# shenweichen/DeepCTR

Hardware: NVIDIA H100
Metric: samples/sec fwd+bwd DeepFM Criteo-synth (higher is better)
Workload: dtype f32

## Files before the change

deepctr_b200/csrc/embed.cu:

```cuda
#include <stdlib.h>
#include <cuda_bf16.h>
#include "common.cuh"

namespace b2ctr {

namespace farm {
__host__ __device__ constexpr uint64_t k0() { return 0xc3a5c85c97cb3127ULL; }
__host__ __device__ constexpr uint64_t k1() { return 0xb492b66fbe98f273ULL; }
__host__ __device__ constexpr uint64_t k2() { return 0x9ae16a3b2f90404fULL; }
__device__ __forceinline__ uint64_t rot(uint64_t v, int s) { return (v >> s) | (v << (64 - s)); }
__device__ __forceinline__ uint64_t shift_mix(uint64_t v) { return v ^ (v >> 47); }
__device__ __forceinline__ uint64_t fetch64(const unsigned char* p) {
  uint64_t r = 0;
#pragma unroll
  for (int i = 7; i >= 0; --i) r = (r << 8) | p[i];
  return r;
}
__device__ __forceinline__ uint64_t fetch32(const unsigned char* p) {
  return (uint64_t)p[0] | ((uint64_t)p[1] << 8) | ((uint64_t)p[2] << 16) | ((uint64_t)p[3] << 24);
}
__device__ __forceinline__ uint64_t hash_len16(uint64_t u, uint64_t v, uint64_t mul) {
  uint64_t a = (u ^ v) * mul;
  a ^= (a >> 47);
  uint64_t b = (v ^ a) * mul;
// ... 212 lines not shown
      V acc = vzero<VEC>();
      bool first = true;
      for (int t0 = 0; t0 < T; t0 += 4) {
        int64_t id[4];
        bool val[4];
        V x[4];
#pragma unroll
        for (int u = 0; u < 4; ++u) {
          const int t = t0 + u;
          id[u] = t < T ? lookup_id(ft, ibase + t) : 0;
          val[u] = t < T && pos_valid(ft, t, id[u], len);
        }
#pragma unroll
        for (int u = 0; u < 4; ++u) {
          const bool need = t0 + u < T && (val[u] || ft.pool == B2CTR_POOL_MAX);
          const bool ok = id_in_range(id[u], ft.vocab);
          if (need && !ok && e == 0) note_oob(fb.oob);
          x[u] = (need && ok) ? vload(ft.table + id[u] * dim + e, (V*)nullptr) : vzero<VEC>();
        }
#pragma unroll
        for (int u = 0; u < 4; ++u) {
          const int t = t0 + u;
          if (t >= T) break;
          V v = x[u];
          if (ft.weight_mode != B2CTR_WEIGHT_NONE) v = vmuls(v, pos_weight(ft, si, b, t, val[u]));
          if (ft.pool == B2CTR_POOL_MAX) {
            if (!val[u]) v = vsubs(v, 1e9f);
            acc = first ? v : vmax(acc, v);
            first = false;
          } else if (val[u]) {
            acc = vadd(acc, v);
          }
        }
      }
      if (ft.pool == B2CTR_POOL_MEAN) acc = vdivs(acc, __fadd_rn(si.L, 1e-8f));
      vstore(out + e, acc);
    }
  }
}

template <int G, int VEC>
__global__ void __launch_bounds__(256)
    embed_scatter_generic_kernel(const __grid_constant__ FeatBlock fb, int64_t batch, float scale) {
  using V = typename VecT<VEC>::T;
  constexpr int kGroups = 256 / G;
  const int lane = threadIdx.x % G;
  const unsigned gmask = G >= 32 ? 0xffffffffu : (((1u << (G & 31)) - 1u) << ((threadIdx.x & 31) / G * G));
  const int64_t ntasks = batch * fb.nfeat;
  for (int64_t task = (int64_t)blockIdx.x * kGroups + threadIdx.x / G; task < ntasks;
       task += (int64_t)gridDim.x * kGroups) {
    const int64_t b = task / fb.nfeat;
    const b2ctr_feature_t& ft = fb.f[task - b * fb.nfeat];
    const int dim = ft.dim, T = ft.maxlen;
    const float* gout = ft.out + b * ft.out_ld + ft.out_col;
    const int64_t ibase = b * ft.idx_stride;

    if (ft.pool == B2CTR_POOL_NONE) {
      for (int t = 0; t < T; ++t) {
        const int64_t id = lookup_id(ft, ibase + t);
        if (!id_in_range(id, ft.vocab)) continue;
        bool nz = false;
        for (int e = lane * VEC; e < dim; e += G * VEC) nz |= vnonzero(vload(gout + (int64_t)t * dim + e, (V*)nullptr));
        if (__ballot_sync(gmask, nz) == 0u) continue;
        float* row = ft.table + id * dim;
        for (int e = lane * VEC; e < dim; e += G * VEC)
          vred(row + e, vmuls(vload(gout + (int64_t)t * dim + e, (V*)nullptr), scale));
      }
      continue;
    }
    const int len = ft.mask_mode == B2CTR_MASK_LENGTH ? ft.len[b * lstride(ft)] : 0;
    const SeqInfo si = seq_info(ft, b);
    for (int e = lane * VEC; e < dim; e += G * VEC) {
      V g = vmuls(vload(gout + e, (V*)nullptr), scale);
      if (ft.pool == B2CTR_POOL_MEAN) g = vdivs(g, __fadd_rn(si.L, 1e-8f));
      if (ft.pool == B2CTR_POOL_MAX) {
        float gv[VEC], mx[VEC];
        int cnt[VEC];
        {
          float tmp[VEC];
          *reinterpret_cast<V*>(tmp) = g;
#pragma unroll
          for (int i = 0; i < VEC; ++i) { gv[i] = tmp[i]; mx[i] = -INFINITY; cnt[i] = 0; }
        }
        for (int pass = 0; pass < 2; ++pass) {
          for (int t = 0; t < T; ++t) {
            const int64_t id = lookup_id(ft, ibase + t);
            const bool valid = pos_valid(ft, t, id, len);
            const bool ok = id_in_range(id, ft.vocab);
            V xv = ok ? vload((ft.src_table ? ft.src_table : ft.table) + id * dim + e, (V*)nullptr) : vzero<VEC>();
            const float w = pos_weight(ft, si, b, t, valid);
            if (ft.weight_mode != B2CTR_WEIGHT_NONE) xv = vmuls(xv, w);
            if (!valid) xv = vsubs(xv, 1e9f);
            float xs[VEC];
            *reinterpret_cast<V*>(xs) = xv;
            if (pass == 0) {
#pragma unroll
              for (int i = 0; i < VEC; ++i) {
                if (xs[i] > mx[i]) { mx[i] = xs[i]; cnt[i] = 1; }
                else if (xs[i] == mx[i]) cnt[i]++;
              }
            } else {
#pragma unroll
              for (int i = 0; i < VEC; ++i)
                if (xs[i] == mx[i] && ok) red_add_f1(ft.table + id * dim + e + i, gv[i] / (float)cnt[i] * w);
            }
          }
        }
        continue;
      }
      for (int t = 0; t < T; ++t) {
        const int64_t id = lookup_id(ft, ibase + t);
        const bool valid = pos_valid(ft, t, id, len);
        if (!valid || !id_in_range(id, ft.vocab)) continue;
        V gt = g;
        if (ft.weight_mode != B2CTR_WEIGHT_NONE) gt = vmuls(gt, pos_weight(ft, si, b, t, true));
        vred(ft.table + id * dim + e, gt);
      }
    }
  }
}

constexpr int kUniMaxFeat = 64;
struct UniParams {
  float* table[kUniMaxFeat];
  float* lin[kUniMaxFeat];
  const void* idx[kUniMaxFeat];
  int64_t idx_stride[kUniMaxFeat];
  int64_t vocab[kUniMaxFeat];
  unsigned long long* oob;
  const float* dense;
  float* x;
  float* linear;
  float* fm;
  int64_t ldx;
  int64_t dense_ld;
  int64_t x_cols;
  uint64_t fm_mask;
  int32_t nfeat;
  int32_t ndense;
  int32_t dim;
  int32_t idx_dtype;
  int32_t has_lin;
  int32_t l2_hints;
  int32_t store_grads;
  float* const* peer_tab;
  float* const* peer_lin;
  int32_t world;
  int32_t wshift;
  __nv_bfloat16* xp_hi;
  __nv_bfloat16* xp_lo;
  int64_t xp_pitch;
};

__device__ __forceinline__ void store_planes4(const UniParams& p, int64_t off, float4 v) {
  const __nv_bfloat16 h0 = __float2bfloat16_rn(v.x), h1 = __float2bfloat16_rn(v.y);
  const __nv_bfloat16 h2 = __float2bfloat16_rn(v.z), h3 = __float2bfloat16_rn(v.w);
  const __nv_bfloat16 l0 = __float2bfloat16_rn(v.x - __bfloat162float(h0));
  const __nv_bfloat16 l1 = __float2bfloat16_rn(v.y - __bfloat162float(h1));
  const __nv_bfloat16 l2 = __float2bfloat16_rn(v.z - __bfloat162float(h2));
  const __nv_bfloat16 l3 = __float2bfloat16_rn(v.w - __bfloat162float(h3));
  uint2 h, l;
  h.x = (uint32_t)__bfloat16_as_ushort(h0) | ((uint32_t)__bfloat16_as_ushort(h1) << 16);
  h.y = (uint32_t)__bfloat16_as_ushort(h2) | ((uint32_t)__bfloat16_as_ushort(h3) << 16);
  l.x = (uint32_t)__bfloat16_as_ushort(l0) | ((uint32_t)__bfloat16_as_ushort(l1) << 16);
  l.y = (uint32_t)__bfloat16_as_ushort(l2) | ((uint32_t)__bfloat16_as_ushort(l3) << 16);
  *reinterpret_cast<uint2*>(p.xp_hi + off) = h;
  *reinterpret_cast<uint2*>(p.xp_lo + off) = l;
}

__device__ __forceinline__ float4 ld_peer_f4(const float* p) {
  float4 r;
  asm volatile("ld.global.L1::no_allocate.v4.f32 {%0,%1,%2,%3}, [%4];"
               : "=f"(r.x), "=f"(r.y), "=f"(r.z), "=f"(r.w)
               : "l"(p));
  return r;
}
__device__ __forceinline__ float ld_peer_f1(const float* p) {
  float r;
  asm volatile("ld.global.L1::no_allocate.f32 %0, [%1];" : "=f"(r) : "l"(p));
  return r;
}
__device__ __forceinline__ void red_peer_f4(float* p, float4 v) {
  asm volatile("red.relaxed.sys.global.add.v4.f32 [%0], {%1,%2,%3,%4};" ::"l"(p), "f"(v.x), "f"(v.y), "f"(v.z),
               "f"(v.w)
               : "memory");
}
__device__ __forceinline__ void red_peer_f1(float* p, float v) {
  asm volatile("red.relaxed.sys.global.add.f32 [%0], %1;" ::"l"(p), "f"(v) : "memory");
}
__device__ __forceinline__ float* shard_row(float* const* tabs, const UniParams& p, int f, int64_t id, int width) {
  const int64_t own = id & (int64_t)(p.world - 1);
  return tabs[(int64_t)f * p.world + own] + (id >> p.wshift) * width;
}

__device__ __forceinline__ int64_t uni_id(const UniParams& p, int f, int64_t b) {
  return load_idx(p.idx[f], b * p.idx_stride[f], p.idx_dtype);
}

template <int LPR, bool SHARD, bool PLANES>
__global__ void __launch_bounds__(256, (SHARD || PLANES) ? 3 : 4)
    gather_uniform_fwd_kernel(const __grid_constant__ UniParams p, int64_t batch) {
  constexpr int RPI = 32 / LPR;
  constexpr int U = 7;
  const int lane = threadIdx.x & 31;
  const int slot = lane / LPR, chunk = lane % LPR;
  const int F = p.nfeat, dim = p.dim;
  const bool hints = p.l2_hints != 0;
  const uint64_t pol_keep = l2_policy_evict_last(), pol_stream = l2_policy_evict_first();
  const int64_t nwarps = (int64_t)gridDim.x * (blockDim.x >> 5);
  int64_t b = (int64_t)blockIdx.x * (blockDim.x >> 5) + (threadIdx.x >> 5);
  auto checked = [&](int f, int64_t bb) -> int64_t {
    if (bb >= batch || f >= F) return 0;
    const int64_t id = uni_id(p, f, bb);
    if (id_in_range(id, p.vocab[f])) return id;
    note_oob(p.oob);
    return -1;
  };
  int64_t id0 = checked(lane, b);
  int64_t id1 = checked(lane + 32, b);
  for (; b < batch; b += nwarps) {
    const int64_t bn = b + nwarps;
    const int64_t nid0 = checked(lane, bn);
    const int64_t nid1 = checked(lane + 32, bn);
    float* xrow = p.x + b * p.ldx;
    float4 s = make_float4(0.f, 0.f, 0.f, 0.f);
    float q = 0.f;
    for (int f0 = 0; f0 < F; f0 += U * RPI) {
      float4 v[U];
#pragma unroll
      for (int u = 0; u < U; ++u) {
        const int f = f0 + u * RPI + slot;
        const int fs = f < F ? f : 0;
        const int64_t ida = __shfl_sync(0xffffffffu, id0, fs & 31);
        const int64_t idb = __shfl_sync(0xffffffffu, id1, fs & 31);
        const int64_t id = fs < 32 ? ida : idb;
        if (f < F) {
          if (id < 0) {
            v[u] = make_float4(0.f, 0.f, 0.f, 0.f);
          } else if (SHARD) {
            v[u] = ld_peer_f4(shard_row(p.peer_tab, p, f, id, dim) + chunk * 4);
          } else {
            const float* src = p.table[f] + id * dim + chunk * 4;
            v[u] = hints ? ldg_stream_f4_pol(src, pol_stream) : ldg_stream_f4(src);
          }
        }
      }
#pragma unroll
      for (int u = 0; u < U; ++u) {
        const int f = f0 + u * RPI + slot;
        if (f < F) {
          if (hints) stg_stream_f4_pol(xrow + (int64_t)f * dim + chunk * 4, v[u], pol_stream);
          else stg_stream_f4(xrow + (int64_t)f * dim + chunk * 4, v[u]);
          if (PLANES) store_planes4(p, b * p.xp_pitch + (int64_t)f * dim + chunk * 4, v[u]);
          if ((p.fm_mask >> f) & 1ull) {
            s.x += v[u].x; s.y += v[u].y; s.z += v[u].z; s.w += v[u].w;
            q += v[u].x * v[u].x + v[u].y * v[u].y + v[u].z * v[u].z + v[u].w * v[u].w;
          }
        }
      }
    }
    if (p.fm != nullptr) {
#pragma unroll
      for (int o = LPR; o < 32; o <<= 1) {
        s.x += __shfl_xor_sync(0xffffffffu, s.x, o);
        s.y += __shfl_xor_sync(0xffffffffu, s.y, o);
        s.z += __shfl_xor_sync(0xffffffffu, s.z, o);
        s.w += __shfl_xor_sync(0xffffffffu, s.w, o);
      }
      float sq = slot == 0 ? (s.x * s.x + s.y * s.y + s.z * s.z + s.w * s.w) : 0.f;
      sq = warp_sum(sq);
      q = warp_sum(q);
      if (lane == 0) p.fm[b] = 0.5f * (sq - q);
    }
    if (p.linear != nullptr) {
      float l = 0.f;
      if (p.has_lin) {
        const bool ok0 = lane < F && id0 >= 0;
        const bool ok1 = lane + 32 < F && id1 >= 0;
        if (SHARD) {
          if (ok0) l += ld_peer_f1(shard_row(p.peer_lin, p, lane, id0, 1));
          if (ok1) l += ld_peer_f1(shard_row(p.peer_lin, p, lane + 32, id1, 1));
        } else {
          if (ok0) l += hints ? ldg_f1_pol(p.lin[lane] + id0, pol_keep) : p.lin[lane][id0];
          if (ok1) l += hints ? ldg_f1_pol(p.lin[lane + 32] + id1, pol_keep) : p.lin[lane + 32][id1];
        }
      }
      l = warp_sum(l);
      if (lane == 0) p.linear[b] = l;
    }
    const int64_t c0 = (int64_t)F * dim;
    for (int64_t c = c0 + lane; c < p.x_cols; c += 32) {
      const int j = (int)(c - c0);
      xrow[c] = j < p.ndense ? p.dense[b * p.dense_ld + j] : 0.f;
    }
    if (PLANES) {
      for (int64_t c = c0 + lane; c < p.xp_pitch; c += 32) {
        const int j = (int)(c - c0);
        const float v = j < p.ndense ? p.dense[b * p.dense_ld + j] : 0.f;
        const __nv_bfloat16 h = __float2bfloat16_rn(v);
        p.xp_hi[b * p.xp_pitch + c] = h;
        p.xp_lo[b * p.xp_pitch + c] = __float2bfloat16_rn(v - __bfloat162float(h));
      }
    }
    id0 = nid0;
    id1 = nid1;
  }
}

template <int LPR, bool SHARD>
__global__ void __launch_bounds__(256, SHARD ? 2 : 3)
    scatter_uniform_bwd_kernel(const __grid_constant__ UniParams p, const float* __restrict__ dx,
                               const float* __restrict__ dfm, const float* __restrict__ dlinear,
                               float scale, float lin_scale, int64_t batch) {
  constexpr int RPI = 32 / LPR;
  constexpr int U = 4;
  const int lane = threadIdx.x & 31;
  const int slot = lane / LPR, chunk = lane % LPR;
  const int F = p.nfeat, dim = p.dim;
  const bool hints = p.l2_hints != 0;
  const uint64_t pol_keep = l2_policy_evict_last(), pol_stream = l2_policy_evict_first();
  const int64_t nwarps = (int64_t)gridDim.x * (blockDim.x >> 5);
  int64_t b = (int64_t)blockIdx.x * (blockDim.x >> 5) + (threadIdx.x >> 5);
  auto checked = [&](int f, int64_t bb) -> int64_t {
    if (bb >= batch || f >= F) return 0;
    const int64_t id = uni_id(p, f, bb);
    return id_in_range(id, p.vocab[f]) ? id : -1;
  };
  int64_t id0 = checked(lane, b);
  int64_t id1 = checked(lane + 32, b);
  for (; b < batch; b += nwarps) {
    const int64_t bn = b + nwarps;
    const int64_t nid0 = checked(lane, bn);
    const int64_t nid1 = checked(lane + 32, bn);
    const float* xrow = p.x + b * p.ldx;
    const float* dxrow = dx ? dx + b * p.ldx : nullptr;
    const float gfm = dfm ? dfm[b] : 0.f;
    float4 s = make_float4(0.f, 0.f, 0.f, 0.f);
    if (dfm) {
      for (int f0 = 0; f0 < F; f0 += U * RPI) {
        float4 v[U];
#pragma unroll
        for (int u = 0; u < U; ++u) {
          const int f = f0 + u * RPI + slot;
          v[u] = make_float4(0.f, 0.f, 0.f, 0.f);
          if (f < F && ((p.fm_mask >> f) & 1ull))
            v[u] = *reinterpret_cast<const float4*>(xrow + (int64_t)f * dim + chunk * 4);
        }
#pragma unroll
        for (int u = 0; u < U; ++u) { s.x += v[u].x; s.y += v[u].y; s.z += v[u].z; s.w += v[u].w; }
      }
#pragma unroll
      for (int o = LPR; o < 32; o <<= 1) {
        s.x += __shfl_xor_sync(0xffffffffu, s.x, o);
        s.y += __shfl_xor_sync(0xffffffffu, s.y, o);
        s.z += __shfl_xor_sync(0xffffffffu, s.z, o);
        s.w += __shfl_xor_sync(0xffffffffu, s.w, o);
      }
    }
    for (int f0 = 0; f0 < F; f0 += U * RPI) {
      float4 g[U], xv[U];
#pragma unroll
      for (int u = 0; u < U; ++u) {
        const int f = f0 + u * RPI + slot;
        g[u] = make_float4(0.f, 0.f, 0.f, 0.f);
        xv[u] = g[u];
        if (f < F) {
          const int64_t off = (int64_t)f * dim + chunk * 4;
          if (dxrow) g[u] = hints ? ldg_stream_f4_pol(dxrow + off, pol_stream) : ldg_stream_f4(dxrow + off);
          if (dfm && ((p.fm_mask >> f) & 1ull)) xv[u] = *reinterpret_cast<const float4*>(xrow + off);
        }
      }
#pragma unroll
      for (int u = 0; u < U; ++u) {
        const int f = f0 + u * RPI + slot;
        const int fs = f < F ? f : 0;
        const int64_t ida = __shfl_sync(0xffffffffu, id0, fs & 31);
        const int64_t idb = __shfl_sync(0xffffffffu, id1, fs & 31);
        const int64_t id = fs < 32 ? ida : idb;
        if (f < F && id >= 0) {
          float4 r = g[u];
          if (dfm && ((p.fm_mask >> f) & 1ull)) {
            r.x += gfm * (s.x - xv[u].x);
            r.y += gfm * (s.y - xv[u].y);
            r.z += gfm * (s.z - xv[u].z);
            r.w += gfm * (s.w - xv[u].w);
          }
          r.x *= scale; r.y *= scale; r.z *= scale; r.w *= scale;
          if (SHARD) red_peer_f4(shard_row(p.peer_tab, p, f, id, dim) + chunk * 4, r);
          else if (p.store_grads) stg_stream_f4(p.table[f] + id * dim + chunk * 4, r);
          else if (hints) red_add_f4_pol(p.table[f] + id * dim + chunk * 4, r, pol_stream);
          else red_add_f4(p.table[f] + id * dim + chunk * 4, r);
        }
      }
    }
    if (dlinear && p.has_lin) {
      const float gl = dlinear[b] * lin_scale;
      const bool ok0 = lane < F && id0 >= 0;
      const bool ok1 = lane + 32 < F && id1 >= 0;
      if (SHARD) {
        if (ok0) red_peer_f1(shard_row(p.peer_lin, p, lane, id0, 1), gl);
        if (ok1) red_peer_f1(shard_row(p.peer_lin, p, lane + 32, id1, 1), gl);
      } else if (p.store_grads) {
        if (ok0) p.lin[lane][id0] = gl;
        if (ok1) p.lin[lane + 32][id1] = gl;
      } else {
        if (ok0) { if (hints) red_add_f1_pol(p.lin[lane] + id0, gl, pol_keep); else red_add_f1(p.lin[lane] + id0, gl); }
        if (ok1) { if (hints) red_add_f1_pol(p.lin[lane + 32] + id1, gl, pol_keep); else red_add_f1(p.lin[lane + 32] + id1, gl); }
      }
    }
    id0 = nid0;
    id1 = nid1;
// ... 335 lines not shown
```

deepctr_b200/inputs.py:

```python
from collections import defaultdict, OrderedDict
from itertools import chain

import ctypes as C

import numpy as np
import torch

from . import _lib as L
from . import kernels as K
from . import engine as E
from .engine import Layer, l2


class Embedding(Layer):
    def __init__(self, input_dim, output_dim, embeddings_initializer=None, embeddings_regularizer=None,
                 mask_zero=False, name=None, **kwargs):
        Layer.__init__(self, name=name, **kwargs)
        self.input_dim, self.output_dim = int(input_dim), int(output_dim)
        self.embeddings_initializer = embeddings_initializer or E.RandomNormal(0.0, 0.05)
        self.embeddings_regularizer = embeddings_regularizer
        self.mask_zero = mask_zero
        self.supports_masking = mask_zero
        self.embeddings = self.add_weight("embeddings", (self.input_dim, self.output_dim),
                                          self.embeddings_initializer, self.embeddings_regularizer,
# ... 371 lines not shown
        self.peers = None

    def _peer_tables(self, fast_slots, lin_fused):
        if self.peers is None:
            from . import parallel
            tabs = [s.emb.embeddings.materialize() for s in fast_slots]
            emb = parallel.PeerTables(self.dist, tabs, L)
            lin = None
            if lin_fused:
                lin = parallel.PeerTables(self.dist, [s.emb.embeddings.materialize().reshape(-1) for s in self.lin], L)
            token = torch.zeros((1,), dtype=torch.float32, device=tabs[0].device)
            self.peers = (emb, lin, token)
        return self.peers

    def _linear_arena(self):
        if getattr(self, "_arena", False) is not False:
            return self._arena
        import os
        self._arena = None
        if os.environ.get("B2CTR_L2_PERSIST", "0") != "1" or getattr(self, "sharded", False):
            return None
        ws, seen = [], set()
        for s_ in self.lin:
            w = s_.emb.embeddings
            if id(w) not in seen:
                seen.add(id(w))
                ws.append(w)
        sizes = [(w.numel() + 63) // 64 * 64 for w in ws]
        total = sum(sizes)
        if total * 4 < (16 << 20) or torch.cuda.is_current_stream_capturing():
            return None
        granted, max_window = K.l2_persist_reserve(total * 4)
        if granted <= 0 or max_window <= 0:
            return None
        arena = torch.empty((total,), dtype=torch.float32, device=ws[0].materialize().device)
        off = 0
        for w, n in zip(ws, sizes):
            view = arena[off:off + w.numel()].view(w.shape_)
            view.copy_(w.materialize())
            w.data = view
            off += n
        nbytes = min(total * 4, max_window)
        self._arena = (arena, (arena.data_ptr(), nbytes, min(1.0, granted / float(nbytes))))
        return self._arena

    def _fast_eligible(self):
        m = self.main
        if not m or len(m) > 64:
            return False
        d = m[0].dim
        if d not in (4, 8, 16, 32, 64, 128):
            return False
        n = 0
        for s in m:
            if s.dim == d and s.maxlen == 1 and s.pool == L.POOL_NONE and s.hash[0] == L.HASH_NONE:
                n += 1
            else:
                break
        self.fast_n = n
        return n >= 1

    def _all_fast_single(self):
        return len(self.main) == self.fast_n and not self.seq and (not self.lin or self._lin_matches_fast())

    def _lin_matches_fast(self):
        if not self.lin or len(self.lin) != self.fast_n or len(self.main) != self.fast_n:
            return False
        for a, b in zip(self.lin, self.main):
            if (a.input_name != b.input_name or a.maxlen != 1 or a.pool != L.POOL_NONE
                    or a.hash[0] != L.HASH_NONE):
                return False
        return True

    def begin_step(self, feed, training):
        self.results = {}
        self.fm_result = self.lin_result = None
        self.tail_done = None
        if not self.slots:
            return
        some = feed[self.slots[0].input_name].data
        batch, dev = some.shape[0], some.device
        grad = training and E.current_tape() is not None
        bufs = {}
        if self.main:
            bufs["main"] = E.Var(torch.empty((batch, self.main_ld), dtype=torch.float32, device=dev),
                                 ncols=self.main_width, owner=self)
        lin_fused = self.fast and self.lin_hint and self._lin_matches_fast()
        if self.lin and not lin_fused:
            bufs["lin"] = E.Var(torch.empty((batch, self.lin_ld), dtype=torch.float32, device=dev),
                                ncols=self.lin_width, owner=self)
        generic = []
        for s in self.slots:
            if s.buf == "seq":
                bufs[id(s)] = E.Var(torch.empty((batch, s.maxlen * s.dim), dtype=torch.float32, device=dev),
                                    owner=self)
        fast_slots = self.main[:self.fast_n] if self.fast else []
        for s in self.slots:
            if s in fast_slots or (lin_fused and s.buf == "lin"):
                continue
            generic.append(s)
        tables_used = []
        plan = None
        if fast_slots:
            x = bufs["main"].data
            self.route = None
            peer = None
            if getattr(self, "sharded", False) and getattr(self, "peer_mode", False):
                peer = self._peer_tables(fast_slots, self.fast and self.lin_hint and self._lin_matches_fast())
                feats = [self._feature(s, feed, x, self.main_ld) for s in fast_slots]
                lin_tabs = None
            elif getattr(self, "sharded", False):
                id_feats = [self._feature(s, feed, x, self.main_ld) for s in fast_slots]
                st = self.exchange.route(id_feats, batch)
                dimf = fast_slots[0].dim
                tabs = [s.emb.embeddings.materialize() for s in fast_slots]
                ltabs = [s.emb.embeddings.materialize().reshape(-1) for s in self.lin] if lin_fused else None
                rows, rlin = self.exchange.fetch(st, tabs, ltabs, dimf)
                self.route = (st, tabs, ltabs, dimf)
                pos = st["pos"]
                feats = [K.make_feature(rows, pos[:, f], x, out_col=s.col, out_ld=self.main_ld)
                         for f, s in enumerate(fast_slots)]
                lin_tabs = [rlin] * len(fast_slots) if lin_fused else None
            else:
                feats = [self._feature(s, feed, x, self.main_ld) for s in fast_slots]
                lin_tabs = [s.emb.embeddings.materialize().reshape(-1) for s in self.lin] if lin_fused else None
            only_fast = len(self.main) == self.fast_n
            dense = None
            if only_fast and self.tail_hint is not None and "__dense_pack__" in feed:
                c0, nd = self.tail_hint
                dp = feed["__dense_pack__"].data
                if c0 + nd <= dp.shape[1] and self.main_width + nd <= self.main_ld:
                    dense = dp[:, c0:c0 + nd]
                    self.tail_done = (c0, nd)
            linear = torch.empty((batch,), dtype=torch.float32, device=dev) if lin_fused else None
            fm, fm_mask = None, 0
            if self.fm_hint is not None:
                c0, nc = self.fm_hint
                d = fast_slots[0].dim
                if c0 % d == 0 and nc % d == 0 and c0 + nc <= self.fast_n * d:
                    fm = torch.empty((batch,), dtype=torch.float32, device=dev)
                    for f in range(c0 // d, (c0 + nc) // d):
                        fm_mask |= 1 << f
            arena = self._linear_arena() if (lin_fused and lin_tabs is not None and peer is None
                                             and getattr(self, "route", None) is None) else None
            if arena is not None:
                lin_tabs = [s.emb.embeddings.materialize().reshape(-1) for s in self.lin]
            plan = K.UniformPlan(feats, lin_tabs, dense, x, linear, fm, fm_mask)
            plan.set_window(arena[1] if arena is not None else None)
            plan.g.x_cols = self.main_ld if only_fast else self.fast_n * fast_slots[0].dim
            if peer is not None:
                plan.set_peers(self.dist.world, peer[0].table, peer[1].table if peer[1] is not None else None)
            from . import ops as _ops
            if (only_fast and self.tail_done is not None and batch % 256 == 0 and batch >= 256
                    and _ops.GEMM_PRECISION == L.GEMM_BF16X3 and _ops.PLANE_REUSE and _ops.GATHER_PLANES):
                kd = self.main_width + self.tail_done[1]
                xp = torch.empty((L.lib().b2ctr_planes_bytes(batch, kd),), dtype=torch.uint8, device=dev)
                plan.g.x_planes = xp.data_ptr()
                plan.g.x_planes_cols = kd
                bufs["main"].xplanes = (kd, xp)
            K.embed_gather_uniform_fwd(plan, batch)
            if fm is not None:
                self.fm_result = (self.fm_hint, E.Var(fm.reshape(batch, 1)))
            if linear is not None:
                self.lin_result = E.Var(linear.reshape(batch, 1))
        if generic:
            feats = []
            for s in generic:
                buf = bufs[id(s)] if s.buf == "seq" else bufs[s.buf]
                feats.append(self._feature(s, feed, buf.data, buf.data.stride(0)))
            K.embed_gather_fwd(feats, batch)
        from . import ops
        vlin = E.Var(None, owner=self, name="__virtual_lin__")
        for s in self.slots:
            if s.buf == "lin" and lin_fused:
                base = vlin
                out = E.Var(None, base=base, col0=s.col, ncols=s.dim, owner=self, vshape=(batch, 1, s.dim))
            elif s.buf == "seq":
                base = bufs[id(s)]
                out = ops._window(base, 0, s.maxlen * s.dim, (batch, s.maxlen, s.dim))
            else:
                base = bufs[s.buf]
                out = ops._window(base, s.col, s.dim, (batch, 1, s.dim))
            if s.pool == L.POOL_NONE and s.mask_zero:
                out.mask = E.KMask(ids=[feed[s.input_name].data], hashed=s.hash)
            out.requires_grad = grad and s.emb.embeddings.trainable
            self.results[id(s.node)] = out
            for vn in s.virtual_nodes:
                if vn is not s.node:
                    self.results[id(vn)] = VIRTUAL
        if grad:
            outs = [b for b in bufs.values()]
            if self.fm_result is not None:
                outs.append(self.fm_result[1])
            if self.lin_result is not None:
                outs.append(self.lin_result)
            for o in outs:
                o.requires_grad = True
            tape = E.current_tape()
            tape.record(outs, lambda grads: self._backward(feed, bufs, plan, fast_slots, generic, lin_fused,
                                                           batch))

    def _feature(self, s, feed, out, out_ld, table=None, src_table=None):
        ids = feed[s.input_name].data
        length = feed[s.len_name].data if s.len_name else None
        weight = feed[s.weight_name].data if s.weight_name else None
        if length is not None and length.dtype != torch.int32:
            raise ValueError("sequence lengths must be int32")
        tab = table if table is not None else s.emb.embeddings.materialize()
        shard = s.emb.embeddings.opt_state.get("shard")
        return K.make_feature(tab, ids, out, out_col=s.col if s.buf != "seq" else 0, out_ld=out_ld,
                              maxlen=s.maxlen, pool=s.pool, mask_mode=s.mask_mode, length=length,
                              weight=weight, weight_mode=s.weight_mode, hash_mode=s.hash[0],
                              src_table=src_table, vocab=shard[2] if shard else s.emb.input_dim)

    @staticmethod
    def _target(w, opt):
        if not w.trainable:
            scratch = w.opt_state.get("scratch")
            if scratch is None:
                scratch = w.opt_state["scratch"] = torch.empty_like(w.data)
            return scratch, 0.0
        return _grad_target(w, opt)

    def _backward(self, feed, bufs, plan, fast_slots, generic, lin_fused, batch):
        opt = E.current_opt()
        if fast_slots:
            main = bufs["main"]
            dx = main.grad
            dfm = self.fm_result[1].grad if self.fm_result is not None else None
            dlin = self.lin_result.grad if self.lin_result is not None else None
            if (dx is not None or dfm is not None or dlin is not None) and getattr(self, "route", None) is not None:
                st, tabs, ltabs, dimf = self.route
                dev = main.data.device
                grows = torch.empty((st["n_send"], dimf), dtype=torch.float32, device=dev)
                glin = torch.empty((st["n_send"],), dtype=torch.float32, device=dev) if lin_fused else None
                if dlin is None and glin is not None:
                    K.fill(glin, 0.0)
                pos = st["pos"]
                feats = [K.make_feature(grows, pos[:, f], main.data, out_col=s.col, out_ld=self.main_ld)
                         for f, s in enumerate(fast_slots)]
                bplan = K.UniformPlan(feats, [glin] * len(fast_slots) if lin_fused else None, None, main.data,
                                      None, None, plan.g.fm_mask[0])
                bplan.g.x_cols = plan.g.x_cols
                bplan.g.flags = L.UNIFORM_STORE_GRADS
                K.embed_scatter_uniform_bwd(bplan, dx, None if dfm is None else dfm.reshape(-1).contiguous(),
                                            None if dlin is None else dlin.reshape(-1).contiguous(),
                                            1.0, 1.0, batch)
                lr = opt["optimizer"].lr if opt and opt.get("optimizer") else 0.0
                sc = -lr / self.dist.world
                self.exchange.push(st, tabs, ltabs, dimf, grows, glin, sc, sc)
            elif (dx is not None or dfm is not None or dlin is not None) and plan.g.world > 1:
                from . import parallel
                emb, lin, token = self.peers
                parallel.device_barrier(self.dist, token)
                lr = opt["optimizer"].lr if opt and opt.get("optimizer") else 0.0
                sc = -lr / self.dist.world
                feats = [self._feature(s, feed, main.data, self.main_ld) for s in fast_slots]
                bplan = K.UniformPlan(feats, None, None, main.data, None, None, plan.g.fm_mask[0])
                bplan.g.x_cols = plan.g.x_cols
                bplan.set_peers(self.dist.world, emb.table, lin.table if (lin is not None and lin_fused) else None)
                K.embed_scatter_uniform_bwd(bplan, dx, None if dfm is None else dfm.reshape(-1).contiguous(),
                                            None if dlin is None else dlin.reshape(-1).contiguous(),
                                            sc, sc, batch)
            elif dx is not None or dfm is not None or dlin is not None:
                tgts = [self._target(s.emb.embeddings, opt) for s in fast_slots]
                feats = [self._feature(s, feed, main.data, self.main_ld, table=tgt)
                         for s, (tgt, _) in zip(fast_slots, tgts)]
                scale = max(abs(sc) for _, sc in tgts) * (-1.0 if any(sc < 0 for _, sc in tgts) else 1.0)
                lin_tabs, lin_scale = None, 0.0
                if lin_fused:
                    lt = [self._target(s.emb.embeddings, opt) for s in self.lin]
                    lin_tabs = [t.reshape(-1) for t, _ in lt]
                    lin_scale = max(abs(sc) for _, sc in lt) * (-1.0 if any(sc < 0 for _, sc in lt) else 1.0)
                bplan = K.UniformPlan(feats, lin_tabs, None, main.data, None, None, plan.g.fm_mask[0])
                bplan.g.x_cols = plan.g.x_cols
                if getattr(self, "sorted_update", False) and all(sc < 0 for _, sc in tgts):
                    o = opt["optimizer"]
                    adagrad = o.name == "adagrad"
                    acc = lacc = None
                    if adagrad:
                        acc = [self._adagrad_state(s.emb.embeddings) for s in fast_slots]
                        lacc = [self._adagrad_state(s.emb.embeddings).reshape(-1) for s in self.lin] if lin_fused else None
                    K.embed_update_sorted(bplan, dx, None if dfm is None else dfm.reshape(-1).contiguous(),
                                          None if dlin is None else dlin.reshape(-1).contiguous(),
                                          1 if adagrad else 0, o.lr, o.lr, 1e-7, acc, lacc, batch)
                    return self._backward_generic(feed, bufs, generic, opt, batch)
                arena = getattr(self, "_arena", None)
                if arena and lin_tabs is not None and all(sc < 0 for _, sc in lt):
                    bplan.set_window(arena[1])
                K.embed_scatter_uniform_bwd(bplan, dx, None if dfm is None else dfm.reshape(-1).contiguous(),
                                            None if dlin is None else dlin.reshape(-1).contiguous(),
                                            scale, lin_scale, batch)
        self._backward_generic(feed, bufs, generic, opt, batch)

    @staticmethod
    def _adagrad_state(w):
        acc = w.opt_state.get("acc")
        if acc is None:
            acc = w.opt_state["acc"] = torch.empty_like(w.data)
            K.fill(acc, 0.1)
        return acc

    def _backward_generic(self, feed, bufs, generic, opt, batch):
        feats, scales = [], []
        flat = {}
        for s in generic:
            if not s.emb.embeddings.trainable:
# ... 402 lines not shown
```

deepctr_b200/ops.py:

```python
import numpy as np
import torch

from . import _lib as L
from . import kernels as K
from . import engine as E

GEMM_PRECISION = L.GEMM_BF16X3


PLANE_REUSE = True
GATHER_PLANES = False


UNCAPTURABLE = 0


def mark_uncapturable():
    global UNCAPTURABLE
    UNCAPTURABLE += 1


def set_gemm_precision(mode):
    global GEMM_PRECISION
    GEMM_PRECISION = {"fp32": L.GEMM_FP32, "bf16x3": L.GEMM_BF16X3}[mode]


def _empty(shape, like):
    return torch.empty(shape, dtype=torch.float32, device=like.device)


def _split_k(m_out, n_out, kred):
    if kred < 4096:
        return 1
    if n_out <= 8:
        blocks = (m_out + 63) // 64
        return int(max(1, min(592 // blocks, kred // 256)))
    tiles = ((m_out + 255) // 256) * ((n_out + 255) // 256)
    return int(max(1, min(74 // tiles if tiles <= 74 else 1, kred // 1024)))


def _as2d(x):
    t2, ld = x.as2d()
    if t2 is None:
        t = E.contiguous(x)
        t2 = t.reshape(-1, t.shape[-1])
        ld = t2.stride(0)
    return t2, ld


def _planes_of(var, t2):
    base = var.base
    if (base is not None and base.xplanes is not None and var.col0 == 0 and base.data is not None
            and base.xplanes[0] == t2.shape[1] and t2.data_ptr() == base.data.data_ptr()
            and t2.stride(0) == base.data.stride(0)):
        return base.xplanes[1]
    key = (t2.data_ptr(), tuple(t2.shape), t2.stride(0))
    if var.planes is None or var.planes[0] != key:
        var.planes = (key, K.split_planes(t2))
    return var.planes[1]


def dense(x, w, b=None, activation=None):
    act = L.ACT_BY_NAME.get(activation, None)
    fused_act = act if act is not None else L.ACT_NONE
    x2, _ = _as2d(x)
    m, kdim = x2.shape
    n = w.shape[1]
    wd = w.materialize() if isinstance(w, E.Weight) else w.data
    bd = (b.materialize() if isinstance(b, E.Weight) else b.data) if b is not None else None
    prec = GEMM_PRECISION if min(n, kdim) >= 16 else L.GEMM_FP32
    reuse = prec == L.GEMM_BF16X3 and PLANE_REUSE and m >= 128
    xp = _planes_of(x, x2) if reuse else None
    wp = K.split_planes(wd) if reuse else None
    y = K.gemm(x2, wd, bias=bd, act=fused_act, precision=prec, m=m, n=n, k=kdim, a_planes=xp, b_planes=wp)
    out = E.Var(y.reshape(tuple(x.data.shape[:-1]) + (n,)))
    if act is None and activation is not None:
        raise ValueError("activation %r cannot be fused into dense(); apply it as a layer" % activation)

    def bwd(grads):
        dy = grads[0].reshape(m, n)
        if not dy.is_contiguous():
            dy = dy.contiguous()
        need_db = b is not None and b.requires_grad
        need_planes = reuse and (x.requires_grad or w.requires_grad)
        dzp = None
        if fused_act != L.ACT_NONE or need_db:
            if need_planes and fused_act != L.ACT_NONE and dy.stride(0) % 4 == 0 and K.planes_fusable(m, n):
                dz, db, dzp = K.bias_act_bwd(dy, y, fused_act, want_dz=True, want_dbias=need_db, want_planes=True)
            else:
                dz, db = K.bias_act_bwd(dy, y, fused_act, want_dz=fused_act != L.ACT_NONE, want_dbias=need_db)
            if dz is None:
                dz = dy
        else:
            dz, db = dy, None
        if need_planes and dzp is None:
            dzp = K.split_planes(dz)
        if x.requires_grad:
            base = x.base
            if (base is not None and x.col0 == 0 and x.ncols != -1 and base.data.dim() == 2
                    and base.data.shape[0] == m and x.ncols == kdim):
                ld = base.data.stride(0)
                buf = _empty((m, ld), dy)
                dxw = buf[:, :kdim]
                K.gemm(dz, wd, c=dxw, trans_b=True, precision=prec, m=m, n=kdim, k=n, a_planes=dzp,
                       b_planes=wp)
                E.add_grad(x, dxw)
            else:
                dx = K.gemm(dz, wd, trans_b=True, precision=prec, m=m, n=kdim, k=n, a_planes=dzp,
                            b_planes=wp)
                E.add_grad(x, dx.reshape(x.data.shape))
        if w.requires_grad:
            dw = K.gemm(x2, dz, trans_a=True, precision=prec, split_k=_split_k(kdim, n, m),
                        m=kdim, n=n, k=m, a_planes=xp, b_planes=dzp)
            E.add_grad(w, dw)
        if need_db:
            E.add_grad(b, db)

    E.record([out], [x, w, b], bwd)
    return out


def activation(x, name):
    act = L.ACT_BY_NAME[name]
    if act == L.ACT_NONE:
        return x
    xt = E.contiguous(x)
    y = K.act_fwd(xt, act)
    out = E.Var(y)

    def bwd(grads):
        dz, _ = K.bias_act_bwd(grads[0].reshape(-1, y.shape[-1]).contiguous(), y.reshape(-1, y.shape[-1]),
                               act, want_dz=True, want_dbias=False)
        E.add_grad(x, dz.reshape(x.data.shape))

    E.record([out], [x], bwd)
    return out


def _window(base, col0, ncols, shape, mask=None):
    bt = base.data
    b = bt.shape[0]
    dense_strides = []
    acc = 1
    for s in reversed(shape[1:]):
        dense_strides.append(acc)
        acc *= s
    dense_strides = list(reversed(dense_strides))
    data = bt.as_strided((b,) + tuple(shape[1:]), (bt.stride(0),) + tuple(dense_strides),
                         bt.storage_offset() + col0)
    return E.Var(data, requires_grad=base.requires_grad, mask=mask, base=base, col0=col0, ncols=ncols,
                 owner=base.owner)


def flatten(x):
    b = x.data.shape[0]
    w = int(np.prod(x.data.shape[1:]))
    if x.base is not None and x.ncols != -1:
        return _window(x.base, x.col0, x.ncols, (b, w))
    t = E.contiguous(x)
    out = E.Var(t.reshape(b, w))
    out.base, out.col0, out.ncols = x if x.base is None else x.base, 0, -1
    out.requires_grad = x.requires_grad
    return out


def reshape(x, shape):
    b = x.data.shape[0]
    shape = (b,) + tuple(shape[1:])
    if x.base is not None and x.ncols != -1:
        return _window(x.base, x.col0, x.ncols, shape, x.mask)
    t = E.contiguous(x)
    out = E.Var(t.reshape(shape), mask=x.mask)
    out.base, out.col0, out.ncols = x if x.base is None else x.base, 0, -1
    out.requires_grad = x.requires_grad
    return out


def _flat_concat_ok(shapes, axis):
    nd = len(shapes[0])
    ax = axis if axis >= 0 else nd + axis
    return ax, all(all(s[d] == 1 for d in range(1, ax)) for s in shapes)


def concat(xs, axis=-1):
    xs = list(xs)
    if len(xs) == 1:
        return xs[0]
    shapes = [tuple(v.shape) for v in xs]
    ax, flat_ok = _flat_concat_ok(shapes, axis)
    out_shape = list(shapes[0])
    out_shape[ax] = sum(s[ax] for s in shapes)
    b = shapes[0][0]
    widths = [int(np.prod(s[1:])) for s in shapes]
    if flat_ok:
        base = xs[0].base
        if base is not None and xs[0].ncols != -1:
            col = xs[0].col0
            ok = True
            for v, w in zip(xs, widths):
                if v.base is not base or v.ncols == -1 or v.col0 != col or v.ncols != w:
                    ok = False
                    break
                col += w
            if ok and base.data is None:
                return E.Var(None, base=base, col0=xs[0].col0, ncols=col - xs[0].col0, owner=base.owner,
                             vshape=tuple(out_shape))
            if ok:
                return _window(base, xs[0].col0, col - xs[0].col0, tuple(out_shape))
    if any(v.data is None for v in xs):
        raise L.B2ctrError("a fused-away (virtual) embedding output reached a layer that needs its values")
    if flat_ok:
        out = _empty((b, sum(widths)), xs[0].data)
        col = 0
        for v, w in zip(xs, widths):
            src, ld = v.flat2d()
            if src is None:
                src = E.contiguous(v).reshape(b, w)
                ld = w
            K.copy2d(src, ld, out, out.stride(0), b, w, dst_off=col)
            col += w
        res = E.Var(out.reshape(out_shape))

        def bwd(grads):
            g = grads[0].reshape(b, -1)
            c = 0
            for v, w in zip(xs, widths):
                if v.requires_grad:
                    gv = _empty((b, w), g)
                    K.copy2d(g, g.stride(0), gv, w, b, w, src_off=c)
                    E.add_grad(v, gv.reshape(v.data.shape))
                c += w

        E.record([res], xs, bwd)
        return res
    lead = int(np.prod(shapes[0][:ax]))
    tails = [int(np.prod(s[ax:])) for s in shapes]
    out = _empty((lead, sum(tails)), xs[0].data)
    col = 0
    for v, w in zip(xs, tails):
        t = E.contiguous(v).reshape(lead, w)
        K.copy2d(t, w, out, out.stride(0), lead, w, dst_off=col)
# ... 405 lines not shown
    z = _empty((chunk * D, kmax), x2)
    ws = [_wdata(f).reshape(-1, f.shape[-1]) for f in filters]
    bs = [_wdata(bv) for bv in biases]
    oc = 0
    for i, size in enumerate(layer_size):
        h = hs[i]
        kdim = m * h
        y = _empty((B * D, size), x2)
        src, vk = (x2, v0) if i == 0 else (ys[-1], (D * layer_size[i - 1], 1, layer_size[i - 1]))
        for b0 in range(0, B, chunk):
            nb = min(chunk, B - b0)
            zc = z.reshape(-1)[:nb * D * kdim].reshape(nb * D, kdim)
            K.cin_outer_fwd(x2, v0, src, vk, zc, b0, nb, m, h, D)
            K.gemm(zc, ws[i], c=y[b0 * D:(b0 + nb) * D], bias=bs[i], act=act, precision=GEMM_PRECISION,
                   m=nb * D, n=size, k=kdim)
        K.cin_sum_d(y, size, direct[i][0], direct[i][1], D, out, out_cols, oc, 0, B)
        oc += direct[i][1]
        ys.append(y)
    res = E.Var(out)

    def bwd(grads):
        with K.profile_tag("cin"):
            _bwd(grads)

    def _bwd(grads):
        g = grads[0]
        if not g.is_contiguous():
            g = g.contiguous()
        dx = _empty((B, m * D), x2)
        K.fill(dx, 0.0)
        gx = (m * D, D, 1)
        dh = None
        col = out_cols
        for i in range(nl - 1, -1, -1):
            size, h = layer_size[i], hs[i]
            kdim = m * h
            col -= direct[i][1]
            dy = _empty((B * D, size), x2)
            K.cin_expand_grad(g, out_cols, col, direct[i][0], direct[i][1], dh, hs[i + 1] if dh is not None else 0,
                              hs[i + 1] if dh is not None else 0, dy, size, D, 0, B)
            dz_, db = K.bias_act_bwd(dy, ys[i], act, want_dz=act != L.ACT_NONE, want_dbias=True)
            if dz_ is None:
                dz_ = dy
            E.add_grad(biases[i], db)
            src, vk = (x2, v0) if i == 0 else (ys[i - 1], (D * layer_size[i - 1], 1, layer_size[i - 1]))
            dhid = None
            if i > 0:
                dhid = _empty((B * D, h), x2)
            dw = _empty((kdim, size), x2)
            K.fill(dw, 0.0)
            for b0 in range(0, B, chunk):
                nb = min(chunk, B - b0)
                zc = z.reshape(-1)[:nb * D * kdim].reshape(nb * D, kdim)
                K.cin_outer_fwd(x2, v0, src, vk, zc, b0, nb, m, h, D)
                dzc = dz_[b0 * D:(b0 + nb) * D]
                K.gemm(zc, dzc, c=dw, trans_a=True, accumulate=True, precision=GEMM_PRECISION,
                       m=kdim, n=size, k=nb * D)
                dzf = K.gemm(dzc, ws[i], c=zc, trans_b=True, precision=GEMM_PRECISION, m=nb * D, n=kdim, k=size)
                if i == 0:
                    K.cin_outer_bwd(dzf, x2, v0, src, vk, dx, gx, True, dx, gx, True, b0, nb, m, h, D)
                else:
                    K.cin_outer_bwd(dzf, x2, v0, src, vk, dx, gx, True, dhid, (D * h, 1, h), False, b0, nb,
                                    m, h, D)
            E.add_grad(filters[i], dw.reshape(filters[i].shape))
            dh = dhid
        E.add_grad(x, dx.reshape(x.shape))

    E.record([res], [x] + list(filters) + list(biases), bwd)
    return res


def interacting_attention(q, k, v, res, heads, dhead, scaling):
    B, F, HD = q.shape
    qt, kt, vt = E.contiguous(q), E.contiguous(k), E.contiguous(v)
    rt = E.contiguous(res) if res is not None else None
    out = K.interacting_fwd(qt, kt, vt, rt, B, F, heads, dhead, scaling)
    o = E.Var(out)

    def bwd(grads):
        g = grads[0]
        if not g.is_contiguous():
            g = g.contiguous()
        dq, dk, dv, dres = K.interacting_bwd(qt, kt, vt, out, g, res is not None, B, F, heads, dhead, scaling)
        E.add_grad(q, dq)
        E.add_grad(k, dk)
        E.add_grad(v, dv)
        if res is not None:
            E.add_grad(res, dres)

    E.record([o], [q, k, v, res], bwd)
    return o


def din_att_input(query, keys):
    B, T, Edim = keys.shape
    qt, ldq = query.flat2d()
    if qt is None:
        qt = E.contiguous(query).reshape(B, Edim)
        ldq = Edim
    kt, ldk = keys.flat2d()
    if kt is None:
        kt = E.contiguous(keys).reshape(B, T * Edim)
        ldk = T * Edim
    out = K.din_att_input_fwd(qt, ldq, kt, ldk, B, T, Edim)
    res = E.Var(out)

    def bwd(grads):
        g = grads[0]
        if not g.is_contiguous():
            g = g.contiguous()
        dq, dk = K.din_att_input_bwd(qt, ldq, kt, ldk, g, B, T, Edim)
        E.add_grad(query, dq.reshape(query.shape))
        E.add_grad(keys, dk.reshape(keys.shape))

    E.record([res], [query, keys], bwd)
    return res


DIN_FUSED = True


def din_att_fusable(query, keys, n_out):
    B, T, Edim = keys.shape
    return (DIN_FUSED and GEMM_PRECISION == L.GEMM_BF16X3 and Edim % 8 == 0 and B * T >= 256 and n_out >= 8
            and n_out % 4 == 0)


def din_att_first(query, keys, w, b, activation):
    B, T, Edim = keys.shape
    qt, ldq = query.flat2d()
    if qt is None or ldq % 4 or qt.data_ptr() % 16:
        qt = E.contiguous(query).reshape(B, Edim)
        ldq = Edim
    kt, ldk = keys.flat2d()
    if kt is None or ldk % 4 or kt.data_ptr() % 16:
        kt = E.contiguous(keys).reshape(B, T * Edim)
        ldk = T * Edim
    act = L.ACT_BY_NAME[activation]
    wd, bd = _wdata(w), (_wdata(b) if b is not None else None)
    n = wd.shape[1]
    wp = K.split_planes(wd)
    y = K.att_gemm(0, qt, ldq, kt, ldk, B, T, Edim, n, wp, bias=bd, act=act)
    out = E.Var(y.reshape(B, T, n))
    rows = B * T

    def bwd(grads):
        dy = grads[0].reshape(rows, n)
        if not dy.is_contiguous():
            dy = dy.contiguous()
        need_db = b is not None and b.requires_grad
        dzp = None
        if act != L.ACT_NONE or need_db:
            if act != L.ACT_NONE and K.planes_fusable(rows, n):
                dz, db, dzp = K.bias_act_bwd(dy, y, act, want_dz=True, want_dbias=need_db, want_planes=True)
            else:
                dz, db = K.bias_act_bwd(dy, y, act, want_dz=act != L.ACT_NONE, want_dbias=need_db)
            if dz is None:
                dz = dy
        else:
            dz, db = dy, None
        if dzp is None:
            dzp = K.split_planes(dz)
        if w.requires_grad:
            dw = K.att_gemm(1, qt, ldq, kt, ldk, B, T, Edim, n, dzp, split_k=_split_k(4 * Edim, n, rows))
            E.add_grad(w, dw)
        if need_db:
            E.add_grad(b, db)
        if query.requires_grad or keys.requires_grad:
            da = K.gemm(dz, wd, trans_b=True, precision=L.GEMM_BF16X3, m=rows, n=4 * Edim, k=n, a_planes=dzp, b_planes=wp)
            dq, dk = K.din_att_input_bwd(qt, ldq, kt, ldk, da, B, T, Edim)
            E.add_grad(query, dq.reshape(query.shape))
            E.add_grad(keys, dk.reshape(keys.shape))

    E.record([out], [query, keys, w, b], bwd)
    return out


def din_attention_pool(score, keys, mask_u8, weight_normalization, return_score):
    B, T, Edim = keys.shape
    st = E.contiguous(score).reshape(B, T)
    kt, ldk = keys.flat2d()
    if kt is None:
        kt = E.contiguous(keys).reshape(B, T * Edim)
        ldk = T * Edim
    out, w = K.din_pool_fwd(st, kt, ldk, mask_u8, B, T, Edim, weight_normalization, return_score)
    res = E.Var(out)

    def bwd(grads):
        g = grads[0]
        if not g.is_contiguous():
            g = g.contiguous()
        dscore, dkeys = K.din_pool_bwd(w, kt, ldk, mask_u8, g, B, T, Edim, weight_normalization, return_score,
                                       want_dkeys=keys.requires_grad)
        E.add_grad(score, dscore.reshape(score.shape))
        if dkeys is not None:
            E.add_grad(keys, dkeys.reshape(keys.shape))

    E.record([res], [score, keys], bwd)
    return res


def _len_i32(lengths):
    t = lengths.data
    if t.dtype != torch.int32:
        raise ValueError("sequence lengths must be int32")
    return dense_i32(t).reshape(-1)


def dense_i32(t):
    if t.is_contiguous():
        return t
    t2 = t.reshape(t.shape[0], -1) if t.dim() != 2 else t
    out = torch.empty(t2.shape, dtype=torch.int32, device=t.device)
    K.copy2d(t2.view(torch.float32), t2.stride(0), out.view(torch.float32), out.stride(0), t2.shape[0], t2.shape[1])
    return out


def seqpool(seq, mode, mask_u8=None, lengths=None):
    B, T, Edim = seq.shape
    xt = E.contiguous(seq)
    ln = _len_i32(lengths) if lengths is not None else None
    code = L.POOL_BY_NAME[mode]
    out = K.seqpool_fwd(xt, mask_u8, ln, B, T, Edim, code)
    res = E.Var(out)

    def bwd(grads):
        g = grads[0]
        if not g.is_contiguous():
            g = g.contiguous()
        E.add_grad(seq, K.seqpool_bwd(xt, mask_u8, ln, g, B, T, Edim, code))

    E.record([res], [seq], bwd)
    return res


def weighted_seq(seq, weights, normalize, mask_u8=None, lengths=None):
    B, T, Edim = seq.shape
    xt = E.contiguous(seq)
    wt_in = E.contiguous(weights).reshape(B, T)
    ln = _len_i32(lengths) if lengths is not None else None
    wt = K.seqweight(wt_in, mask_u8, ln, B, T, normalize)
    out = K.seqscale(xt, wt, B * T, Edim)
    res = E.Var(out, mask=seq.mask)

    def bwd(grads):
        g = grads[0]
        if not g.is_contiguous():
            g = g.contiguous()
        E.add_grad(seq, K.seqscale(g, wt, B * T, Edim))

    E.record([res], [seq], bwd)
    return res


def _stats_for(x2, m, n, mean_w, var_w, training, momentum):
    if training:
        stats = K.colstats(x2, n, m, n)
        K.moving_update(mean_w.materialize(), stats[0], momentum)
        K.moving_update(var_w.materialize(), stats[1], momentum)
        return stats[0], stats[1]
    return mean_w.materialize(), var_w.materialize()


def dice(x, alphas, moving_mean, moving_var, eps, training, momentum=0.99):
    xt = E.contiguous(x)
    n = xt.shape[-1]
    m = xt.numel() // n
    x2 = xt.reshape(m, n)
    mean, var = _stats_for(x2, m, n, moving_mean, moving_var, training, momentum)
    al = alphas.materialize()
    y = K.dice_fwd(x2, mean, var, al, m, n, eps)
    res = E.Var(y.reshape(xt.shape))

    def bwd(grads):
        g = grads[0].reshape(m, n)
        if not g.is_contiguous():
            g = g.contiguous()
        dx, dalpha = K.dice_bwd(x2, mean, var, al, g, m, n, eps, training)
        E.add_grad(x, dx.reshape(x.shape))
        E.add_grad(alphas, dalpha)

    E.record([res], [x, alphas], bwd)
    return res


def batchnorm(x, gamma, beta, moving_mean, moving_var, eps, training, momentum=0.99):
    xt = E.contiguous(x)
    n = xt.shape[-1]
    m = xt.numel() // n
    x2 = xt.reshape(m, n)
    mean, var = _stats_for(x2, m, n, moving_mean, moving_var, training, momentum)
    gd = gamma.materialize() if gamma is not None else None
    bd = beta.materialize() if beta is not None else None
    y = K.bn_apply(x2, mean, var, gd, bd, m, n, eps)
    res = E.Var(y.reshape(xt.shape))

    def bwd(grads):
        g = grads[0].reshape(m, n)
        if not g.is_contiguous():
            g = g.contiguous()
        dx, dgamma, dbeta = K.bn_bwd(x2, mean, var, gd, g, m, n, eps, training)
        E.add_grad(x, dx.reshape(x.shape))
        if gamma is not None:
            E.add_grad(gamma, dgamma)
        if beta is not None:
            E.add_grad(beta, dbeta)

# ... 33 lines not shown
```

Measured before the change: 31.53 million.

## Enable fused gather-time bf16 plane emission and skip redundant dz materialization

```diff
diff --git a/deepctr_b200/csrc/embed.cu b/deepctr_b200/csrc/embed.cu
--- a/deepctr_b200/csrc/embed.cu
+++ b/deepctr_b200/csrc/embed.cu
@@ -388,7 +388,8 @@
   int64_t xp_pitch;
 };
 
-__device__ __forceinline__ void store_planes4(const UniParams& p, int64_t off, float4 v) {
+template <int LPR>
+__device__ __forceinline__ void store_planes4(const UniParams& p, int64_t off, float4 v, bool ok) {
   const __nv_bfloat16 h0 = __float2bfloat16_rn(v.x), h1 = __float2bfloat16_rn(v.y);
   const __nv_bfloat16 h2 = __float2bfloat16_rn(v.z), h3 = __float2bfloat16_rn(v.w);
   const __nv_bfloat16 l0 = __float2bfloat16_rn(v.x - __bfloat162float(h0));
@@ -400,8 +401,18 @@
   h.y = (uint32_t)__bfloat16_as_ushort(h2) | ((uint32_t)__bfloat16_as_ushort(h3) << 16);
   l.x = (uint32_t)__bfloat16_as_ushort(l0) | ((uint32_t)__bfloat16_as_ushort(l1) << 16);
   l.y = (uint32_t)__bfloat16_as_ushort(l2) | ((uint32_t)__bfloat16_as_ushort(l3) << 16);
-  *reinterpret_cast<uint2*>(p.xp_hi + off) = h;
-  *reinterpret_cast<uint2*>(p.xp_lo + off) = l;
+  if constexpr (LPR >= 2) {
+    const bool odd = threadIdx.x & 1;
+    const uint32_t gx = __shfl_xor_sync(0xffffffffu, odd ? h.x : l.x, 1);
+    const uint32_t gy = __shfl_xor_sync(0xffffffffu, odd ? h.y : l.y, 1);
+    if (ok) {
+      if (odd) *reinterpret_cast<uint4*>(p.xp_lo + off - 4) = make_uint4(gx, gy, l.x, l.y);
+      else *reinterpret_cast<uint4*>(p.xp_hi + off) = make_uint4(h.x, h.y, gx, gy);
+    }
+  } else if (ok) {
+    *reinterpret_cast<uint2*>(p.xp_hi + off) = h;
+    *reinterpret_cast<uint2*>(p.xp_lo + off) = l;
+  }
 }
 
 __device__ __forceinline__ float4 ld_peer_f4(const float* p) {
@@ -434,10 +445,10 @@
 }
 
 template <int LPR, bool SHARD, bool PLANES>
-__global__ void __launch_bounds__(256, (SHARD || PLANES) ? 3 : 4)
+__global__ void __launch_bounds__(256, SHARD ? 3 : 4)
     gather_uniform_fwd_kernel(const __grid_constant__ UniParams p, int64_t batch) {
   constexpr int RPI = 32 / LPR;
-  constexpr int U = 7;
+  constexpr int U = PLANES ? 5 : 7;
   const int lane = threadIdx.x & 31;
   const int slot = lane / LPR, chunk = lane % LPR;
   const int F = p.nfeat, dim = p.dim;
@@ -470,10 +481,9 @@
         const int64_t ida = __shfl_sync(0xffffffffu, id0, fs & 31);
         const int64_t idb = __shfl_sync(0xffffffffu, id1, fs & 31);
         const int64_t id = fs < 32 ? ida : idb;
-        if (f < F) {
-          if (id < 0) {
-            v[u] = make_float4(0.f, 0.f, 0.f, 0.f);
-          } else if (SHARD) {
+        v[u] = make_float4(0.f, 0.f, 0.f, 0.f);
+        if (f < F && id >= 0) {
+          if (SHARD) {
             v[u] = ld_peer_f4(shard_row(p.peer_tab, p, f, id, dim) + chunk * 4);
           } else {
             const float* src = p.table[f] + id * dim + chunk * 4;
@@ -487,12 +497,12 @@
         if (f < F) {
           if (hints) stg_stream_f4_pol(xrow + (int64_t)f * dim + chunk * 4, v[u], pol_stream);
           else stg_stream_f4(xrow + (int64_t)f * dim + chunk * 4, v[u]);
-          if (PLANES) store_planes4(p, b * p.xp_pitch + (int64_t)f * dim + chunk * 4, v[u]);
           if ((p.fm_mask >> f) & 1ull) {
             s.x += v[u].x; s.y += v[u].y; s.z += v[u].z; s.w += v[u].w;
             q += v[u].x * v[u].x + v[u].y * v[u].y + v[u].z * v[u].z + v[u].w * v[u].w;
           }
         }
+        if (PLANES) store_planes4<LPR>(p, b * p.xp_pitch + (int64_t)f * dim + chunk * 4, v[u], f < F);
       }
     }
     if (p.fm != nullptr) {
diff --git a/deepctr_b200/inputs.py b/deepctr_b200/inputs.py
--- a/deepctr_b200/inputs.py
+++ b/deepctr_b200/inputs.py
@@ -547,7 +547,7 @@
                 plan.set_peers(self.dist.world, peer[0].table, peer[1].table if peer[1] is not None else None)
             from . import ops as _ops
             if (only_fast and self.tail_done is not None and batch % 256 == 0 and batch >= 256
-                    and _ops.GEMM_PRECISION == L.GEMM_BF16X3 and _ops.PLANE_REUSE and _ops.GATHER_PLANES):
+                    and _ops.GEMM_PRECISION == L.GEMM_BF16X3 and _ops.PLANE_REUSE):
                 kd = self.main_width + self.tail_done[1]
                 xp = torch.empty((L.lib().b2ctr_planes_bytes(batch, kd),), dtype=torch.uint8, device=dev)
                 plan.g.x_planes = xp.data_ptr()
diff --git a/deepctr_b200/ops.py b/deepctr_b200/ops.py
--- a/deepctr_b200/ops.py
+++ b/deepctr_b200/ops.py
@@ -9,7 +9,6 @@
 
 
 PLANE_REUSE = True
-GATHER_PLANES = False
 
 
 UNCAPTURABLE = 0
@@ -86,7 +85,8 @@
         dzp = None
         if fused_act != L.ACT_NONE or need_db:
             if need_planes and fused_act != L.ACT_NONE and dy.stride(0) % 4 == 0 and K.planes_fusable(m, n):
-                dz, db, dzp = K.bias_act_bwd(dy, y, fused_act, want_dz=True, want_dbias=need_db, want_planes=True)
+                _, db, dzp = K.bias_act_bwd(dy, y, fused_act, want_dz=False, want_dbias=need_db, want_planes=True)
+                dz = dy
             else:
                 dz, db = K.bias_act_bwd(dy, y, fused_act, want_dz=fused_act != L.ACT_NONE, want_dbias=need_db)
             if dz is None:
@@ -798,7 +798,8 @@
         dzp = None
         if act != L.ACT_NONE or need_db:
             if act != L.ACT_NONE and K.planes_fusable(rows, n):
-                dz, db, dzp = K.bias_act_bwd(dy, y, act, want_dz=True, want_dbias=need_db, want_planes=True)
+                _, db, dzp = K.bias_act_bwd(dy, y, act, want_dz=False, want_dbias=need_db, want_planes=True)
+                dz = dy
             else:
                 dz, db = K.bias_act_bwd(dy, y, act, want_dz=act != L.ACT_NONE, want_dbias=need_db)
             if dz is None:
```

New measurement: 33.35 million (median of 6 runs). 5.8% higher.
